# AlejandroSilvestri/os1

Measured on AMD Instinct MI355X. Metric: frames/sec extract+match, 1920x1080 @ 2000 ORB feats, higher is better.
Workload: dtype u8

## Files before the change

### os1_amd/csrc/orbfe_extractor.hip

```cpp
#include <hip/hip_runtime.h>
#include <unistd.h>
#include <sched.h>

#include <algorithm>
#include <cctype>
#include <chrono>
#include <cmath>
#include <cstdarg>
#include <cstdio>
#include <cstdlib>
#include <cstring>
#include <memory>
#include <mutex>
#include <string>
#include <thread>
#include <vector>

#include "../../include/orbfe.h"
#include "glibc_sincosf.h"
#include "host_pool.h"
#include "orbfe_internal.h"
#include "quadtree.h"

namespace orbfe {
int launch_pyramid(const PyramidParams& P, int nframes, hipStream_t st, const ConeParams* cone);
void launch_ingest(const uint8_t* src, long long sstride, uint8_t* dst, long long dpitch, int rowBytes, int rows, hipStream_t st);
void launch_to_gray(const uint8_t* const* raw, long long rawStride, const uint8_t* const* gray, long long grayPitch, int rows,
                    int cols, int channels, const int coef[3], int shift, bool aligned, int nframes, hipStream_t st);
void launch_fast(const PyramidParams& P, int nframes, hipStream_t st);
uint32_t fast_cell_geo(int wCell, int hCell);
void launch_compact(const PyramidParams& P, int nframes, hipStream_t st);
void launch_compact_local(const PyramidParams& P, int nframes, hipStream_t st, int level0, int level1);
void launch_describe(const PyramidParams& P, const SelKp* sel, int nsel, float* angle, uint8_t* desc,
                     hipStream_t st);
void launch_sincos(const float* deg, int n, float* c, float* s, hipStream_t st);
void launch_spin(unsigned long long ticks, hipStream_t st);
void launch_describe_slots(const PyramidParams& P, const SelKp* sel, int nslots, float* angle, uint8_t* desc,
                           const uint32_t* selCount, int selPerFrame, const int* selOff, hipStream_t st, bool fourWaves, float* angle2 = nullptr,
                           uint8_t* desc2 = nullptr);
int launch_quadtree(const QtParams& Q, int nframes, hipStream_t st, int ldsBudget);
int bow_launch_descend(orbfe_vocabulary* v, const uint8_t* d_desc, int n, int levelsup, uint2* d_out, hipStream_t st);
int bow_assemble(orbfe_vocabulary* v, const uint2* ln, int n, uint32_t* bow_ids, double* bow_values, int* n_words,
                 uint32_t* fv_nodes, uint32_t* fv_offsets, uint32_t* fv_features, int* n_fv_nodes,
                 uint32_t* word_of_feature, uint32_t* node_of_feature);
int bow_device(const orbfe_vocabulary* v);
void launch_sfi(const SfiParams& S, int nframes, hipStream_t st);
void launch_sfi_carry(const SfiParams& S, int lastFrame, SelKp* cSel, float* cAngle, uint8_t* cDesc, uint32_t* cCount,
                      hipStream_t st);

thread_local std::string g_err;
void set_err(const char* fmt, ...) {
  char buf[512];
  va_list ap;
  va_start(ap, fmt);
  vsnprintf(buf, sizeof buf, fmt, ap);
  va_end(ap);
  g_err = buf;
}
}

using namespace orbfe;

#define HIP_TRY(expr)                                                                        \
  do {                                                                                       \
    hipError_t e_ = (expr);                                                                  \
    if (e_ != hipSuccess) {                                                                  \
      set_err("%s failed: %s (%s:%d)", #expr, hipGetErrorString(e_), __FILE__, __LINE__);    \
      return ORBFE_ERR_HIP;                                                                  \
    }                                                                                        \
  } while (0)

namespace {
inline int cv_round_f(float v) { return (int)lrintf(v); }
inline int cv_floor_f(float v) { int i = (int)v; return i - (i > v); }
inline short sat_short(int v) { return (short)(v < -32768 ? -32768 : v > 32767 ? 32767 : v); }
inline long long align_up(long long v, long long a) { return (v + a - 1) / a * a; }
double now_ms() {
  return std::chrono::duration<double, std::milli>(std::chrono::steady_clock::now().time_since_epoch()).count();
}

template <class T>
struct DevBuf {
  T* p = nullptr;
  size_t n = 0;
  int ensure(size_t count) {
    if (count <= n) return ORBFE_OK;
    if (p) (void)hipFree(p);
    p = nullptr;
    n = 0;
    HIP_TRY(hipMalloc((void**)&p, count * sizeof(T)));
    n = count;
    return ORBFE_OK;
  }
  void release() { if (p) (void)hipFree(p); p = nullptr; n = 0; }
};
template <class T>
struct PinBuf {
  T* p = nullptr;
  size_t n = 0;
  int ensure(size_t count) {
    if (count <= n) return ORBFE_OK;
    if (p) (void)hipHostFree(p);
    p = nullptr;
    n = 0;
    HIP_TRY(hipHostMalloc((void**)&p, count * sizeof(T), hipHostMallocDefault));
    n = count;
    return ORBFE_OK;
  }
  void release() { if (p) (void)hipHostFree(p); p = nullptr; n = 0; }
};
}

struct orbfe_sfi_chain {
  int device = 0, n0cap = 0;
  DevBuf<SelKp> sel[2];
  DevBuf<float> angle[2];
  DevBuf<uint8_t> desc[2];
  DevBuf<uint32_t> count;
  hipEvent_t ready[2] = {};
  long long seq = 0;
  bool isolated = false;
  bool restart = false;
  orbfe_matcher* hostMatcher = nullptr;
  std::vector<OrbfeKeyPoint> hostPrevKps;
  std::vector<uint8_t> hostPrevDesc;
  bool hostPrevValid = false;
  ~orbfe_sfi_chain() {
    (void)hipSetDevice(device);
    if (hostMatcher) orbfe_matcher_destroy(hostMatcher);
    for (int i = 0; i < 2; i++) { sel[i].release(); angle[i].release(); desc[i].release(); if (ready[i]) (void)hipEventDestroy(ready[i]); }
    count.release();
  }
};

struct UploadLane {
  std::mutex mu;
  hipStream_t stream = nullptr;
};
static UploadLane* upload_lane(int device) {
  static std::mutex mu;
  static UploadLane* lanes[64] = {};
  if (device < 0 || device >= 64) return nullptr;
  std::lock_guard<std::mutex> lk(mu);
  if (!lanes[device]) {
    UploadLane* l = new UploadLane;
    if (hipStreamCreateWithFlags(&l->stream, hipStreamNonBlocking) != hipSuccess) { delete l; return nullptr; }
    lanes[device] = l;
  }
  return lanes[device];
}

struct orbfe_extractor {
  int nfeatures, nlevels, iniTh, minTh, device;
  double scaleFactor;
  std::vector<float> sf, isf, sigma2, isigma2;
  std::vector<int> nfeat;
  static constexpr int kMaxSub = 4;
  hipStream_t stream = nullptr;
  hipStream_t streams[kMaxSub] = {};
  static constexpr int subBatches = 4;
  hipEvent_t evUpload = nullptr;
  bool lastLocalCand = false, submitLocalCand = false;
  bool localLists = true;
  hipEvent_t evFrame0 = nullptr, evS1[kMaxSub] = {};
  int subSel[kMaxSub] = {};
  size_t candHostCap = 0;
  bool gpuQuadtree = true;
  orbfe_vocabulary* voc = nullptr;
  int vocLevelsup = 4;
  bool pendingBow = false;
  DevBuf<uint2> d_bow;
  PinBuf<uint2> h_bow;
  std::vector<std::vector<uint2>> bowKp;
  int kpPerFrameCap = 0;
  bool geomGpuQtOk = true;
  QtParams QP{};
  int selOff[kMaxLevels + 1] = {};
  int selPerFrame = 0;
  DevBuf<uint16_t> d_own;
  hipEvent_t evQt[2] = {};
  std::vector<int> frameKpBase, frameKpCount;

  int rows = 0, cols = 0, batchCap = 0;
  PyramidParams P{};
  DevBuf<uint8_t> d_tables, d_slab, d_in;
  DevBuf<ConeRange> d_coneTab, d_coneTailTab;
  ConeParams coneTail{};
  bool tailOk = false;
  int tailBase = 0, tailTile = 48;
  ConeParams cone{};
  bool coneOk = false;
  bool qtJump = true;
  int qtLdsBudget = 120 * 1024;
  int pollWaitUs = 0;
  bool zeroCopyOut = true;
  bool zeroCopyBatches = false;
  bool ingestKernel = true;
  int coneTile = 0;
  int coneMaxFrames = 2;
  DevBuf<FastCell> d_cells;
  DevBuf<uint8_t> d_zeros;
  DevBuf<uint32_t> d_cellCount, d_slots, d_cand;
  DevBuf<const uint8_t*> d_frame0;
  template <class T> struct View { T* p = nullptr; };
  DevBuf<uint8_t> d_outArena;
  PinBuf<uint8_t> h_outArena;
  size_t outArenaBytes = 0;
  View<uint32_t> d_levelStart, d_selCount, h_levelStart, h_selCount;
  View<SelKp> d_sel, h_sel;
  View<float> d_angle, h_angle;
  View<uint8_t> d_desc, h_desc;
  View<int32_t> d_m12, h_m12, d_nm, h_nm;
  DevBuf<uint16_t> d_sfiOrder;
  DevBuf<int> d_sfiOrderCount;
  DevBuf<uint32_t> d_sfiPool, d_sfiPcount;
  bool pendingMatched = false;
  DevBuf<float> d_f32tmp;
  bool profileKernels = false;
  PinBuf<const uint8_t*> h_frame0;
  PinBuf<uint32_t> h_cand;
  long long inPitch = 0;
  int inFormat = ORBFE_INPUT_GRAY8, grayVariant = ORBFE_GRAY_Q15;
  int gaussVariant = ORBFE_GAUSS_ED;
  long long grayPitch = 0;
  DevBuf<uint8_t> d_gray;
  bool inLinear = false;
  int lastFrames = 0;
  int deferredFrames = 0, deferredCap = 0;
  bool deferredMatched = false;
  std::vector<OrbfeKeyPoint> defKps;
  std::vector<uint8_t> defDesc;
  std::vector<int> defN, defNm;
  std::vector<int32_t> defM12;
  bool lastGpuQt = false, lastZeroCopy = false, submitZeroCopy = false;
  bool describe4 = true;
  float stageMs[5] = {0, 0, 0, 0, 0};
  hipEvent_t ev[kMaxSub][6] = {};
  double kernMs[5] = {0, 0, 0, 0, 0};
  long long kernBatches = 0, kernFrames = 0;

  struct Meta { int16_t x, y; uint8_t score, level; };
  struct Worker {
    QuadTree qt;
    std::vector<int16_t> qx, qy;
    std::vector<uint8_t> qs;
    std::vector<int> qsel;
  };
  std::unique_ptr<HostPool> pool;
  int hostThreads = 1;
  std::vector<Worker> workers;
  std::vector<std::vector<Meta>> taskOut;
  std::vector<Meta> meta;

  ~orbfe_extractor() {
    (void)hipSetDevice(device);
    for (auto& st : streams) if (st) (void)hipStreamSynchronize(st);
    d_bow.release(); h_bow.release();
    d_tables.release(); d_coneTab.release(); d_coneTailTab.release(); d_slab.release(); d_in.release(); d_cellCount.release();
    d_sfiOrder.release(); d_sfiOrderCount.release(); d_sfiPool.release(); d_sfiPcount.release();
    d_cells.release(); d_zeros.release(); d_slots.release(); d_cand.release(); d_frame0.release(); d_gray.release(); d_outArena.release(); h_outArena.release();
    d_f32tmp.release();
    h_frame0.release(); h_cand.release();
    for (auto& es : ev) for (auto& e : es) if (e) (void)hipEventDestroy(e);
    for (auto& e : evS1) if (e) (void)hipEventDestroy(e);
    for (auto& e : evQt) if (e) (void)hipEventDestroy(e);
    d_own.release();
    if (evFrame0) (void)hipEventDestroy(evFrame0);
    if (evUpload) (void)hipEventDestroy(evUpload);

    for (auto& st : streams) if (st) (void)hipStreamDestroy(st);
  }

  int setGeometry(int r, int c) {
    if (r == rows && c == cols) return ORBFE_OK;
    if (c > 4095 || r > 4095) {
      set_err("image %dx%d exceeds the 4095-pixel coordinate packing limit", c, r);
      return ORBFE_ERR_INVALID;
    }
    bool qtOk = true;
    int kpSum = 8;
    PyramidParams Q{};
    Q.nlevels = nlevels;
    Q.iniTh = iniTh;
// ... 306 lines not shown
      int g = f + 1;
      while (g < f0 + nf && gray[g] == gray[g - 1] + frameBytes) g++;
      HIP_TRY(hipMemcpyAsync(d_in.p + frameBytes * f, gray[f], frameBytes * (size_t)(g - f - 1) + lastBytes, hipMemcpyHostToDevice, st));
      for (int k = f; k < g; k++) devAt[k] = d_in.p + frameBytes * k;
      f = g;
    }
    return ORBFE_OK;
  }

  int uploadSlots(int f0, int nf, const uint8_t* const* gray, size_t stride, int r, int c, hipStream_t st) {
    for (int f = f0; f < f0 + nf; f++) {
      if (inLinear)
        HIP_TRY(hipMemcpyAsync(d_in.p + (size_t)inPitch * rows * f, gray[f], stride * (size_t)(r - 1) + c, hipMemcpyHostToDevice, st));
      else
        HIP_TRY(hipMemcpy2DAsync(d_in.p + (size_t)inPitch * rows * f, inPitch, gray[f], stride, c, r, hipMemcpyHostToDevice, st));
    }
    return ORBFE_OK;
  }

  int runGpuQt(int nframes, const uint8_t* const* gray, bool onDevice, int r, int c, size_t stride, OrbfeKeyPoint* kps,
               uint8_t* desc, int cap, int* n_out) {
    int rc = submitGpuQt(nframes, gray, onDevice, r, c, stride);
    if (rc) return rc;
    return waitGpuQt(kps, desc, cap, n_out);
  }

  bool submitProfiled = false, fastTimed = false;
  std::vector<const uint8_t*> devAt;
  int pendingFrames = 0;
  double tSubmit0 = 0, tSubmit1 = 0;

  struct MatchSpec { orbfe_sfi_chain* chain; float bounds[4]; int window; float nnratio; int checkOri; };

  int submitGpuQt(int nframes, const uint8_t* const* gray, bool onDevice, int r, int c, size_t stride,
                  const MatchSpec* ms = nullptr) {
    if (pendingFrames) { set_err("a submitted batch has not been collected yet"); return ORBFE_ERR_INVALID; }
    HIP_TRY(hipSetDevice(device));
    int rc;
    if ((rc = setGeometry(r, c))) return rc;
    if (!geomGpuQtOk) {
      set_err("image %dx%d: a pyramid level has more than 4 (or no) quadtree root nodes; only the blocking "
              "orbfe_extract / orbfe_extract_batch calls (host quadtree path) handle such aspect ratios", c, r);
      return ORBFE_ERR_INVALID;
    }
    if ((rc = setBatch(nframes, !onDevice, stride))) return rc;
    const double t0 = now_ms();
    hipStream_t st = streams[0];
    const int ch = inChannels();
    const int rowBytes = c * ch;
    for (int f = 0; f < nframes; f++)
      if (!gray[f]) { set_err("frame %d is NULL", f); return ORBFE_ERR_INVALID; }
    devAt.resize(nframes);
    bool pinned = !onDevice;
    std::vector<const uint8_t*>& mappedAt = devAt;
    if (!onDevice) {
      const size_t extent = stride * (size_t)(r - 1) + (size_t)rowBytes;
      const int ncheck = nframes <= coneMaxFrames ? nframes : 1;
      for (int f = 0; f < ncheck && pinned; f++) {
        void* dp = nullptr;
        void* dpEnd = nullptr;
        const bool ok = hipHostGetDevicePointer(&dp, const_cast<uint8_t*>(gray[f]), 0) == hipSuccess && dp &&
                        hipHostGetDevicePointer(&dpEnd, const_cast<uint8_t*>(gray[f]) + extent - 1, 0) == hipSuccess &&
                        (const uint8_t*)dpEnd - (const uint8_t*)dp == (ptrdiff_t)(extent - 1);
        if (!ok) { (void)hipGetLastError(); pinned = false; break; }
        mappedAt[f] = static_cast<const uint8_t*>(dp);
      }
    }
    if (!onDevice && !pinned) {
      if ((rc = uploadFrames(0, nframes, gray, stride, r, rowBytes, st, devAt.data()))) return rc;
    } else if (!onDevice && ingestKernel && nframes <= coneMaxFrames &&
               ((((uintptr_t)gray[0] | (uintptr_t)gray[nframes - 1] | (uintptr_t)stride | (uintptr_t)rowBytes) & 3) == 0)) {
      for (int f = 0; f < nframes; f++) {
        uint8_t* d = d_in.p + (size_t)inPitch * rows * f;
        launch_ingest(mappedAt[f], (long long)stride, d, inPitch, rowBytes, r, st);
        devAt[f] = d;
      }
      HIP_TRY(hipGetLastError());
    } else if (!onDevice) {
      UploadLane* lane = upload_lane(device);
      if (!lane) { set_err("cannot create the upload stream"); return ORBFE_ERR_HIP; }
      std::lock_guard<std::mutex> lk(lane->mu);
      if ((rc = uploadFrames(0, nframes, gray, stride, r, rowBytes, lane->stream, devAt.data()))) return rc;
      HIP_TRY(hipEventRecord(evUpload, lane->stream));
      HIP_TRY(hipStreamWaitEvent(st, evUpload, 0));
    }
    bool rawAligned = ((onDevice ? (long long)stride : inPitch) & 3) == 0;
    for (int f = 0; f < nframes; f++) {
      const uint8_t* raw = onDevice ? gray[f] : devAt[f];
      rawAligned = rawAligned && ((uintptr_t)raw & (ch == 4 ? 15 : 3)) == 0;
      h_frame0.p[f] = ch == 1 ? raw : d_gray.p + (size_t)grayPitch * rows * f;
      h_frame0.p[nframes + f] = raw;
    }
    const long long rawStride = onDevice ? (long long)stride : inPitch;
    P.stride0 = ch == 1 ? rawStride : grayPitch;
    P.frameBase = 0;
    P.gaussVariant = gaussVariant;
    if (ch == 1 && nframes <= 2) {
      P.frame0 = nullptr;
      P.frameInline[0] = h_frame0.p[0];
      P.frameInline[1] = h_frame0.p[nframes - 1];
    } else {
      P.frame0 = d_frame0.p;
      HIP_TRY(hipMemcpyAsync(d_frame0.p, h_frame0.p, sizeof(void*) * nframes * (ch == 1 ? 1 : 2), hipMemcpyHostToDevice, st));
    }
    if (ch > 1) {
      const bool q15 = grayVariant == ORBFE_GRAY_Q15;
      const int cr = q15 ? 9798 : 4899, cg = q15 ? 19235 : 9617, cb = q15 ? 3735 : 1868;
      const bool rgb = inFormat == ORBFE_INPUT_RGB8 || inFormat == ORBFE_INPUT_RGBA8;
      const int coef[3] = {rgb ? cr : cb, cg, rgb ? cb : cr};
      launch_to_gray(d_frame0.p + nframes, rawStride, d_frame0.p, grayPitch, r, c, ch, coef, q15 ? 15 : 14, rawAligned, nframes, st);
    }
    const bool prof = profileKernels;
    QP.cand = d_cand.p; QP.levelStart = d_levelStart.p; QP.candCap = P.candCap; QP.nlevels = nlevels; QP.frameBase = 0;
    QP.own = d_own.p;
    QP.sel = d_sel.p; QP.selCount = d_selCount.p; QP.selPerFrame = selPerFrame;
    const bool small = nframes <= coneMaxFrames;
    const bool zeroCopy = zeroCopyOut && small && !voc && !(ms && ms->chain);
    submitZeroCopy = zeroCopy;
    QP.jump = qtJump ? 1 : 0;
    const bool kernelOut = zeroCopyBatches && !small;
    QP.selHost = (zeroCopy || kernelOut) ? h_sel.p : nullptr;
    QP.selCountHost = (zeroCopy || kernelOut) ? h_selCount.p : nullptr;
    for (int l = 0; l < nlevels; l++) {
      QP.levW[l] = P.lv[l].w; QP.levH[l] = P.lv[l].h; QP.nfeat[l] = nfeat[l]; QP.selOff[l] = selOff[l];
      QP.candBase[l] = P.lv[l].slotBase;
    }
    float* angOut = zeroCopy ? h_angle.p : d_angle.p;
    uint8_t* descOut = zeroCopy ? h_desc.p : d_desc.p;
    const int qtLds = small ? qtLdsBudget : 0;
    const bool four = describe4 && small;
    const bool localCand = small && localLists;
    submitLocalCand = localCand;
    QP.levelLocal = localCand ? 1 : 0;
    {
      if (prof) HIP_TRY(hipEventRecord(ev[0][0], st));
      if (launch_pyramid(P, nframes, st, coneOk && small ? &cone : (tailOk && !small ? &coneTail : nullptr))) { set_err("cannot configure the pyramid kernel"); return ORBFE_ERR_HIP; }
      const bool timeFast = prof || !small;
      fastTimed = timeFast;
      if (timeFast) HIP_TRY(hipEventRecord(ev[0][1], st));
      launch_fast(P, nframes, st);
      if (timeFast) HIP_TRY(hipEventRecord(ev[0][2], st));
      if (localCand) launch_compact_local(P, nframes, st, 0, nlevels);
      else launch_compact(P, nframes, st);
      if (prof) HIP_TRY(hipEventRecord(ev[0][3], st));
      if (prof) HIP_TRY(hipEventRecord(evQt[0], st));
      if (launch_quadtree(QP, nframes, st, qtLds)) { set_err("cannot configure the quadtree kernel"); return ORBFE_ERR_HIP; }
      if (prof) HIP_TRY(hipEventRecord(evQt[1], st));
      if (prof) HIP_TRY(hipEventRecord(ev[0][4], st));
      launch_describe_slots(P, d_sel.p, nframes * selPerFrame, angOut, descOut, d_selCount.p, selPerFrame, selOff, st, four,
                            kernelOut ? h_angle.p : nullptr, kernelOut ? h_desc.p : nullptr);
      if (prof) HIP_TRY(hipEventRecord(ev[0][5], st));
      HIP_TRY(hipGetLastError());
    }
    const int nslots = nframes * selPerFrame;
    pendingBow = false;
    if (voc) {
      if ((rc = d_bow.ensure(nslots)) || (rc = h_bow.ensure(nslots))) return rc;
      if ((rc = bow_launch_descend(voc, d_desc.p, nslots, vocLevelsup, d_bow.p, st))) return rc;
      HIP_TRY(hipMemcpyAsync(h_bow.p, d_bow.p, sizeof(uint2) * nslots, hipMemcpyDeviceToHost, st));
      pendingBow = true;
    }
    pendingMatched = false;
    if (ms && ms->chain) {
      orbfe_sfi_chain& ch = *ms->chain;
      const int n0cap = selOff[1] - selOff[0];
      if (ch.n0cap != n0cap || ch.device != device) { set_err("match chain belongs to a different extractor configuration"); return ORBFE_ERR_INVALID; }
      if ((rc = d_sfiOrder.ensure((size_t)batchCap * n0cap))) return rc;
      if ((rc = d_sfiOrderCount.ensure(batchCap))) return rc;
      if ((rc = d_sfiPool.ensure((size_t)batchCap * n0cap * n0cap))) return rc;
      if ((rc = d_sfiPcount.ensure((size_t)batchCap * n0cap))) return rc;
      SfiParams SP{};
      SP.sel = d_sel.p; SP.angle = d_angle.p; SP.desc = d_desc.p; SP.selCount = d_selCount.p;
      SP.selPerFrame = selPerFrame; SP.n0cap = n0cap; SP.frameBase = 0;
      const int prev = (int)((ch.seq + 1) & 1), cur = (int)(ch.seq & 1);
      SP.carrySel = ch.sel[prev].p; SP.carryAngle = ch.angle[prev].p; SP.carryDesc = ch.desc[prev].p;
      const bool iso = ch.isolated;
      SP.carryCount = ch.count.p + ((ch.seq == 0 || iso || ch.restart) ? 2 : prev);
      ch.restart = false;
      SP.minX = ms->bounds[0]; SP.minY = ms->bounds[2];
      SP.invW = static_cast<float>(64) / static_cast<float>(ms->bounds[1] - ms->bounds[0]);
      SP.invH = static_cast<float>(48) / static_cast<float>(ms->bounds[3] - ms->bounds[2]);
      SP.window = (float)ms->window; SP.nnratio = ms->nnratio; SP.checkOri = ms->checkOri;
      SP.order = d_sfiOrder.p; SP.orderCount = d_sfiOrderCount.p; SP.pool = d_sfiPool.p; SP.pcount = d_sfiPcount.p;
      SP.matches12 = kernelOut ? h_m12.p : d_m12.p; SP.nmatches = kernelOut ? h_nm.p : d_nm.p;
      if (ch.seq > 0 && !iso) HIP_TRY(hipStreamWaitEvent(st, ch.ready[prev], 0));
      launch_sfi(SP, nframes, st);
      HIP_TRY(hipGetLastError());
      if (!iso) {
        launch_sfi_carry(SP, nframes - 1, ch.sel[cur].p, ch.angle[cur].p, ch.desc[cur].p, ch.count.p + cur, st);
        HIP_TRY(hipGetLastError());
        HIP_TRY(hipEventRecord(ch.ready[cur], st));
      }
      ch.seq++;
      pendingMatched = true;
    }
    if (!zeroCopy && !kernelOut) HIP_TRY(hipMemcpyAsync(h_outArena.p, d_outArena.p, outArenaBytes, hipMemcpyDeviceToHost, st));
    submitProfiled = prof;
    tSubmit0 = t0;
    tSubmit1 = now_ms();
    pendingFrames = nframes;
    return ORBFE_OK;
  }

  int waitOnly() {
    if (!pendingFrames) return ORBFE_OK;
    HIP_TRY(hipSetDevice(device));
    hipStream_t st = streams[0];
    if (pollWaitUs > 0) {
      hipError_t q;
      while ((q = hipStreamQuery(st)) == hipErrorNotReady) usleep((useconds_t)pollWaitUs);
      if (q != hipSuccess) HIP_TRY(q);
    }
    HIP_TRY(hipStreamSynchronize(st));
    return ORBFE_OK;
  }

  int waitGpuQt(OrbfeKeyPoint* kps, uint8_t* desc, int cap, int* n_out, int32_t* matches12 = nullptr,
                int* nmatches = nullptr) {
    if (!pendingFrames) { set_err("no submitted batch to collect"); return ORBFE_ERR_INVALID; }
    HIP_TRY(hipSetDevice(device));
    const int nframes = pendingFrames;
    pendingFrames = 0;
    hipStream_t st = streams[0];
    const double t0 = tSubmit0, t1 = tSubmit1;
    const double t1b = now_ms();
    if (pollWaitUs > 0) {
      hipError_t q;
      while ((q = hipStreamQuery(st)) == hipErrorNotReady) usleep((useconds_t)pollWaitUs);
      if (q != hipSuccess) HIP_TRY(q);
    }
    HIP_TRY(hipStreamSynchronize(st));
    const double t2 = now_ms();
    {
      float ms = 0;
      if (fastTimed && hipEventElapsedTime(&ms, ev[0][1], ev[0][2]) == hipSuccess) kernMs[1] += ms;
      if (submitProfiled) {
        if (hipEventElapsedTime(&ms, ev[0][0], ev[0][1]) == hipSuccess) kernMs[0] += ms;
        if (hipEventElapsedTime(&ms, ev[0][2], ev[0][3]) == hipSuccess) kernMs[2] += ms;
        if (hipEventElapsedTime(&ms, ev[0][4], ev[0][5]) == hipSuccess) kernMs[3] += ms;
        if (hipEventElapsedTime(&ms, evQt[0], evQt[1]) == hipSuccess) kernMs[4] += ms;
      }
      if (fastTimed) {
        kernBatches++;
        kernFrames += nframes;
      }
    }
    int status = ORBFE_OK;
    if (pendingBow) bowKp.resize(nframes);
    else bowKp.clear();
    for (int f = 0; f < nframes; f++) {
      OrbfeKeyPoint* ko = kps + (size_t)f * cap;
      uint8_t* dout = desc + (size_t)f * cap * 32;
      if (pendingBow) bowKp[f].clear();
      int n = 0;
      for (int l = 0; l < nlevels; l++) {
        const int cnt = (int)h_selCount.p[(size_t)f * kMaxLevels + l];
        const size_t base = (size_t)f * selPerFrame + selOff[l];
        const float scale = sf[l];
        const float size = (float)(int)(31 * sf[l]);
        for (int i = 0; i < cnt; i++) {
          if (n >= cap) { n++; continue; }
          const SelKp s = h_sel.p[base + i];
          OrbfeKeyPoint kp;
          kp.x = (float)(s.xy & 0xffff);
          kp.y = (float)(s.xy >> 16);
          if (l != 0) { kp.x *= scale; kp.y *= scale; }
          kp.size = size;
          kp.angle = h_angle.p[base + i];
          kp.response = (float)(s.lf >> 24);
          kp.octave = l;
          kp.class_id = -1;
          ko[n] = kp;
          memcpy(dout + (size_t)n * 32, h_desc.p + (base + i) * 32, 32);
          if (pendingBow) bowKp[f].push_back(h_bow.p[base + i]);
          n++;
        }
      }
      n_out[f] = n;
      if (n > cap) {
        set_err("frame %d produced %d keypoints, cap is %d", f, n, cap);
        status = ORBFE_ERR_OVERFLOW;
      }
    }
    if (matches12 && nmatches) {
      const int n0cap = selOff[1] - selOff[0];
      for (int f = 0; f < nframes; f++) {
        int32_t* row = matches12 + (size_t)f * cap;
        const int m = std::min(cap, n0cap);
        if (pendingMatched) {
          memcpy(row, h_m12.p + (size_t)f * n0cap, sizeof(int32_t) * m);
          nmatches[f] = h_nm.p[f];
        } else {
          nmatches[f] = 0;
        }
        for (int i = pendingMatched ? m : 0; i < cap; i++) row[i] = -1;
      }
    }
    const double t3 = now_ms();
    stageMs[0] = (float)(t1 - t0);
    stageMs[1] = (float)(t2 - t1b);
    stageMs[2] = 0;
    stageMs[3] = (float)(t3 - t2);
    stageMs[4] = (float)(t3 - t0);
    lastFrames = nframes;
    lastGpuQt = true;
    lastZeroCopy = submitZeroCopy;
    lastLocalCand = submitLocalCand;
    return status;
  }

  int run(int nframes, const uint8_t* const* gray, bool onDevice, int r, int c, size_t stride, OrbfeKeyPoint* kps,
          uint8_t* desc, int cap, int* n_out) {
    if (pendingFrames) { set_err("a submitted batch has not been collected yet"); return ORBFE_ERR_INVALID; }
    HIP_TRY(hipSetDevice(device));
    int rc;
    if ((rc = setGeometry(r, c))) return rc;
    if ((rc = setBatch(nframes, !onDevice, stride))) return rc;
    const double t0 = now_ms();
    if (!pool) {
      pool.reset(new HostPool(hostThreads));
      workers.resize(hostThreads);
    }
    if (inChannels() != 1) { set_err("colour input needs the GPU quadtree path (unset ORBFE_HOST_QUADTREE)"); return ORBFE_ERR_INVALID; }
    const int nsub = std::min(nframes, std::min(kMaxSub, std::max(1, subBatches)));
    const int maxKp = kpPerFrameCap;
    if ((rc = ensureSubStreams(nsub))) return rc;
    int subF0[kMaxSub + 1];
    for (int s = 0; s <= nsub; s++) subF0[s] = (int)((long long)nframes * s / nsub);

    devAt.resize(nframes);
    for (int f = 0; f < nframes; f++) {
      if (!gray[f]) { set_err("frame %d is NULL", f); return ORBFE_ERR_INVALID; }
      h_frame0.p[f] = onDevice ? gray[f] : d_in.p + (size_t)inPitch * rows * f;
    }
    P.stride0 = onDevice ? (long long)stride : inPitch;
    P.gaussVariant = gaussVariant;
    P.frame0 = d_frame0.p;
    HIP_TRY(hipMemcpyAsync(d_frame0.p, h_frame0.p, sizeof(void*) * nframes, hipMemcpyHostToDevice, streams[0]));
    HIP_TRY(hipEventRecord(evFrame0, streams[0]));
    for (int s = 0; s < nsub; s++) {
      hipStream_t st = streams[s];
      const int f0 = subF0[s], nf = subF0[s + 1] - f0;
      if (s) HIP_TRY(hipStreamWaitEvent(st, evFrame0, 0));
      if (!onDevice && (rc = uploadSlots(f0, nf, gray, stride, r, c, st))) return rc;
      PyramidParams Q = P;
// ... 516 lines not shown
  if (v && !h->gpuQuadtree) { set_err("the fused bag-of-words path needs the GPU quadtree path"); return ORBFE_ERR_INVALID; }
  h->voc = v;
  h->vocLevelsup = levelsup;
  return ORBFE_OK;
}

int orbfe_extract_bow(orbfe_extractor* h, int frame, uint32_t* bow_ids, double* bow_values, int* n_words, uint32_t* fv_nodes,
                      uint32_t* fv_offsets, uint32_t* fv_features, int* n_fv_nodes, uint32_t* word_of_feature,
                      uint32_t* node_of_feature) {
  if (!h || !bow_ids || !bow_values || !n_words || !fv_nodes || !fv_offsets || !fv_features || !n_fv_nodes) {
    set_err("bad argument");
    return ORBFE_ERR_INVALID;
  }
  if (!h->voc || frame < 0 || frame >= (int)h->bowKp.size()) {
    set_err("no bag-of-words result for frame %d (set a vocabulary before extracting)", frame);
    return ORBFE_ERR_INVALID;
  }
  const std::vector<uint2>& ln = h->bowKp[frame];
  return bow_assemble(h->voc, ln.data(), (int)ln.size(), bow_ids, bow_values, n_words, fv_nodes, fv_offsets, fv_features,
                      n_fv_nodes, word_of_feature, node_of_feature);
}

int orbfe_extract_bow_raw(orbfe_extractor* h, int frame, uint32_t* leaf_node, uint32_t* level_node, int cap, int* n_out) {
  if (!h || !leaf_node || !level_node || !n_out || cap < 0) { set_err("bad argument"); return ORBFE_ERR_INVALID; }
  if (!h->voc || frame < 0 || frame >= (int)h->bowKp.size()) {
    set_err("no bag-of-words result for frame %d (set a vocabulary before extracting)", frame);
    return ORBFE_ERR_INVALID;
  }
  const std::vector<uint2>& ln = h->bowKp[frame];
  *n_out = (int)ln.size();
  const int m = std::min(cap, (int)ln.size());
  for (int i = 0; i < m; i++) { leaf_node[i] = ln[i].x; level_node[i] = ln[i].y; }
  return ORBFE_OK;
}

int orbfe_extractor_max_keypoints_for_size(const orbfe_extractor* h, int rows, int cols) {
  if (!h || rows <= 0 || cols <= 0) return 0;
  int n = 0;
  for (int l = 0; l < h->nlevels; l++) {
    const int w = cv_round_f((float)cols * h->isf[l]), hh = cv_round_f((float)rows * h->isf[l]);
    int roots = hh > 2 * kBorder ? (int)roundf(static_cast<float>(w - 2 * kBorder) / (hh - 2 * kBorder)) : 0;
    if (roots < 0) roots = 0;
    n += std::max(h->nfeat[l] + 2, 4 * roots);
  }
  return n;
}

int orbfe_extract_batch(orbfe_extractor* h, int nframes, const uint8_t* const* gray, int in_device_memory, int rows,
                        int cols, size_t stride_bytes, OrbfeKeyPoint* kps, uint8_t* desc, int cap, int* n_out) {
  if (!h || !n_out) { set_err("NULL argument"); return ORBFE_ERR_INVALID; }
  if (nframes <= 0) return ORBFE_OK;
  for (int f = 0; f < nframes; f++) n_out[f] = 0;
  if (rows == 0 || cols == 0 || !gray) return ORBFE_OK;
  if (rows < 0 || cols < 0 || stride_bytes < (size_t)cols * h->inChannels() || !kps || !desc || cap <= 0) {
    set_err("invalid image / output arguments");
    return ORBFE_ERR_INVALID;
  }
  if (h->pendingFrames) { set_err("a submitted batch has not been collected yet"); return ORBFE_ERR_INVALID; }
  {
    HIP_TRY(hipSetDevice(h->device));
    const int rc = h->setGeometry(rows, cols);
    if (rc) return rc;
  }
  if (h->gpuQuadtree && h->geomGpuQtOk)
    return h->runGpuQt(nframes, gray, in_device_memory != 0, rows, cols, stride_bytes, kps, desc, cap, n_out);
  return h->run(nframes, gray, in_device_memory != 0, rows, cols, stride_bytes, kps, desc, cap, n_out);
}

static bool gpu_route_ok(orbfe_extractor* h, int rows, int cols, int* rc) {
  *rc = ORBFE_OK;
  if (!h->gpuQuadtree) return false;
  if (hipSetDevice(h->device) != hipSuccess) { set_err("hipSetDevice failed"); *rc = ORBFE_ERR_HIP; return false; }
  if (h->pendingFrames || h->deferredFrames) return true;
  *rc = h->setGeometry(rows, cols);
  return *rc == ORBFE_OK && h->geomGpuQtOk;
}

static int deferred_extract(orbfe_extractor* h, int nframes, const uint8_t* const* gray, int in_device_memory, int rows, int cols,
                            size_t stride_bytes) {
  if (h->pendingFrames || h->deferredFrames) { set_err("a submitted batch has not been collected yet"); return ORBFE_ERR_INVALID; }
  const int cap = orbfe_extractor_max_keypoints_for_size(h, rows, cols);
  h->deferredCap = cap;
  h->defKps.resize((size_t)nframes * cap);
  h->defDesc.resize((size_t)nframes * cap * 32);
  h->defN.assign(nframes, 0);
  const int rc = orbfe_extract_batch(h, nframes, gray, in_device_memory, rows, cols, stride_bytes, h->defKps.data(), h->defDesc.data(),
                                     cap, h->defN.data());
  if (rc) return rc;
  h->deferredFrames = nframes;
  h->deferredMatched = false;
  return ORBFE_OK;
}

static int deferred_collect(orbfe_extractor* h, OrbfeKeyPoint* kps, uint8_t* desc, int cap, int* n_out, int32_t* matches12,
                            int* nmatches) {
  const int nframes = h->deferredFrames, dcap = h->deferredCap;
  h->deferredFrames = 0;
  int status = ORBFE_OK;
  for (int f = 0; f < nframes; f++) {
    const int n = h->defN[f];
    n_out[f] = n;
    if (n > cap) { set_err("frame %d produced %d keypoints, cap is %d", f, n, cap); status = ORBFE_ERR_OVERFLOW; }
    const int m = std::min(n, cap);
    memcpy(kps + (size_t)f * cap, h->defKps.data() + (size_t)f * dcap, sizeof(OrbfeKeyPoint) * (size_t)m);
    memcpy(desc + (size_t)f * cap * 32, h->defDesc.data() + (size_t)f * dcap * 32, 32 * (size_t)m);
    if (matches12 && nmatches) {
      int32_t* row = matches12 + (size_t)f * cap;
      for (int i = 0; i < cap; i++) row[i] = -1;
      nmatches[f] = 0;
      if (h->deferredMatched) {
        memcpy(row, h->defM12.data() + (size_t)f * dcap, sizeof(int32_t) * (size_t)std::min(cap, dcap));
        nmatches[f] = h->defNm[f];
      }
    }
  }
  return status;
}

int orbfe_extract_batch_submit(orbfe_extractor* h, int nframes, const uint8_t* const* gray, int in_device_memory,
                               int rows, int cols, size_t stride_bytes) {
  if (!h || !gray || nframes <= 0 || rows <= 0 || cols <= 0 || stride_bytes < (size_t)cols * h->inChannels()) {
    set_err("invalid arguments");
    return ORBFE_ERR_INVALID;
  }
  int rc;
  if (!gpu_route_ok(h, rows, cols, &rc)) {
    if (rc) return rc;
    return deferred_extract(h, nframes, gray, in_device_memory, rows, cols, stride_bytes);
  }
  if (h->deferredFrames) { set_err("a submitted batch has not been collected yet"); return ORBFE_ERR_INVALID; }
  return h->submitGpuQt(nframes, gray, in_device_memory != 0, rows, cols, stride_bytes);
}

int orbfe_extract_batch_wait(orbfe_extractor* h) {
  if (!h) { set_err("invalid arguments"); return ORBFE_ERR_INVALID; }
  if (h->deferredFrames) return ORBFE_OK;
  return h->waitOnly();
}

int orbfe_extract_batch_collect(orbfe_extractor* h, OrbfeKeyPoint* kps, uint8_t* desc, int cap, int* n_out) {
  if (!h || !kps || !desc || !n_out || cap <= 0) { set_err("invalid arguments"); return ORBFE_ERR_INVALID; }
  if (h->deferredFrames) return deferred_collect(h, kps, desc, cap, n_out, nullptr, nullptr);
  return h->waitGpuQt(kps, desc, cap, n_out);
}

int orbfe_sfi_chain_create(const orbfe_extractor* h, orbfe_sfi_chain** out) {
  if (!h || !out) { set_err("NULL argument"); return ORBFE_ERR_INVALID; }
  *out = nullptr;
  HIP_TRY(hipSetDevice(h->device));
  orbfe_sfi_chain* c = new orbfe_sfi_chain();
  c->device = h->device;
  c->n0cap = h->selOff[1] - h->selOff[0];
  int rc = ORBFE_OK;
  for (int i = 0; i < 2 && rc == ORBFE_OK; i++) {
    if ((rc = c->sel[i].ensure(c->n0cap))) break;
    if ((rc = c->angle[i].ensure(c->n0cap))) break;
    if ((rc = c->desc[i].ensure((size_t)c->n0cap * 32))) break;
    if (hipEventCreateWithFlags(&c->ready[i], hipEventDisableTiming) != hipSuccess) { set_err("hipEventCreate failed"); rc = ORBFE_ERR_HIP; }
  }
  if (rc == ORBFE_OK) rc = c->count.ensure(4);
  if (rc == ORBFE_OK) {
    const uint32_t init[4] = {0xffffffffu, 0xffffffffu, 0xffffffffu, 0xffffffffu};
    if (hipMemcpy(c->count.p, init, sizeof init, hipMemcpyHostToDevice) != hipSuccess) { set_err("hipMemcpy failed"); rc = ORBFE_ERR_HIP; }
  }
  if (rc != ORBFE_OK) { delete c; return rc; }
  *out = c;
  return ORBFE_OK;
}

void orbfe_sfi_chain_destroy(orbfe_sfi_chain* c) { delete c; }

int orbfe_sfi_chain_set_isolated(orbfe_sfi_chain* c, int isolated) {
  if (!c) { set_err("chain is NULL"); return ORBFE_ERR_INVALID; }
  if (c->isolated != (isolated != 0)) {
    c->seq = 0;
    c->hostPrevValid = false;
  }
  c->isolated = isolated != 0;
  return ORBFE_OK;
}

int orbfe_sfi_chain_restart(orbfe_sfi_chain* c) {
  if (!c) { set_err("chain is NULL"); return ORBFE_ERR_INVALID; }
  c->restart = true;
  return ORBFE_OK;
}

int orbfe_extract_batch_submit_matched(orbfe_extractor* h, orbfe_sfi_chain* chain, int nframes, const uint8_t* const* gray,
                                       int in_device_memory, int rows, int cols, size_t stride_bytes, const float bounds[4],
                                       int window_size, float nnratio, int check_orientation) {
  if (!h || !chain || !gray || !bounds || nframes <= 0 || rows <= 0 || cols <= 0 || stride_bytes < (size_t)cols * h->inChannels() || window_size <= 0) {
    set_err("invalid arguments");
    return ORBFE_ERR_INVALID;
  }
  int rc;
  if (!gpu_route_ok(h, rows, cols, &rc)) {
    if (rc) return rc;
    if ((rc = deferred_extract(h, nframes, gray, in_device_memory, rows, cols, stride_bytes))) return rc;
    if (!chain->hostMatcher && (rc = orbfe_matcher_create(h->device, &chain->hostMatcher))) { h->deferredFrames = 0; return rc; }
    const int cap = h->deferredCap;
    h->defM12.assign((size_t)nframes * cap, -1);
    h->defNm.assign(nframes, 0);
    std::vector<const OrbfeKeyPoint*> k1, k2;
    std::vector<const uint8_t*> d1, d2;
    std::vector<int> n1, n2, frameOf, nm;
    std::vector<std::vector<float>> pxy;
    std::vector<float*> prev;
    std::vector<int32_t*> m12;
    for (int f = 0; f < nframes; f++) {
      const OrbfeKeyPoint* pk;
      const uint8_t* pd;
      int pn;
      if (f == 0) {
        if (!chain->hostPrevValid || chain->isolated || chain->restart) continue;
        pk = chain->hostPrevKps.data(); pd = chain->hostPrevDesc.data(); pn = (int)chain->hostPrevKps.size();
      } else {
        pk = h->defKps.data() + (size_t)(f - 1) * cap; pd = h->defDesc.data() + (size_t)(f - 1) * cap * 32; pn = h->defN[f - 1];
      }
      pxy.emplace_back((size_t)std::max(pn, 1) * 2);
      for (int j = 0; j < pn; j++) { pxy.back()[2 * j] = pk[j].x; pxy.back()[2 * j + 1] = pk[j].y; }
      k1.push_back(pk); d1.push_back(pd); n1.push_back(pn);
      k2.push_back(h->defKps.data() + (size_t)f * cap); d2.push_back(h->defDesc.data() + (size_t)f * cap * 32); n2.push_back(h->defN[f]);
      m12.push_back(h->defM12.data() + (size_t)f * cap);
      frameOf.push_back(f);
    }
    for (auto& v : pxy) prev.push_back(v.data());
    nm.assign(k1.size(), 0);
    if (!k1.empty()) {
      rc = orbfe_search_for_initialization_batch(chain->hostMatcher, (int)k1.size(), k1.data(), d1.data(), n1.data(), k2.data(), d2.data(),
                                                 n2.data(), bounds, prev.data(), m12.data(), window_size, nnratio, check_orientation,
                                                 nm.data());
      if (rc) { h->deferredFrames = 0; return rc; }
      for (size_t p = 0; p < frameOf.size(); p++) h->defNm[frameOf[p]] = nm[p];
    }
    const int last = nframes - 1, ln = h->defN[last];
    chain->hostPrevKps.assign(h->defKps.begin() + (size_t)last * cap, h->defKps.begin() + (size_t)last * cap + ln);
    chain->hostPrevDesc.assign(h->defDesc.begin() + (size_t)last * cap * 32, h->defDesc.begin() + ((size_t)last * cap + ln) * 32);
    chain->hostPrevValid = !chain->isolated;
    chain->restart = false;
    h->deferredMatched = true;
    return ORBFE_OK;
  }
  if (h->deferredFrames) { set_err("a submitted batch has not been collected yet"); return ORBFE_ERR_INVALID; }
  orbfe_extractor::MatchSpec ms;
  ms.chain = chain;
  memcpy(ms.bounds, bounds, sizeof ms.bounds);
  ms.window = window_size;
  ms.nnratio = nnratio;
  ms.checkOri = check_orientation;
  return h->submitGpuQt(nframes, gray, in_device_memory != 0, rows, cols, stride_bytes, &ms);
}

int orbfe_extract_batch_collect_matched(orbfe_extractor* h, OrbfeKeyPoint* kps, uint8_t* desc, int cap, int* n_out,
                                        int32_t* matches12, int* nmatches) {
  if (!h || !kps || !desc || !n_out || !matches12 || !nmatches || cap <= 0) { set_err("invalid arguments"); return ORBFE_ERR_INVALID; }
  if (h->deferredFrames) return deferred_collect(h, kps, desc, cap, n_out, matches12, nmatches);
  return h->waitGpuQt(kps, desc, cap, n_out, matches12, nmatches);
}

int orbfe_extract(orbfe_extractor* h, const uint8_t* gray, int rows, int cols, size_t stride_bytes, OrbfeKeyPoint* kps,
                  uint8_t* desc, int cap, int* n_out) {
  if (!n_out) { set_err("n_out is NULL"); return ORBFE_ERR_INVALID; }
  *n_out = 0;
  if (!gray || rows == 0 || cols == 0) return ORBFE_OK;
  const uint8_t* frames[1] = {gray};
  return orbfe_extract_batch(h, 1, frames, 0, rows, cols, stride_bytes, kps, desc, cap, n_out);
}

int orbfe_debug_level_size(const orbfe_extractor* h, int level, int* w, int* hgt) {
  if (!h || level < 0 || level >= h->nlevels || h->rows == 0) { set_err("bad level / no frame yet"); return ORBFE_ERR_INVALID; }
  *w = h->P.lv[level].w;
  *hgt = h->P.lv[level].h;
  return ORBFE_OK;
}

int orbfe_debug_level_copy(orbfe_extractor* h, int frame, int level, uint8_t* out) {
  if (!h || level < 0 || level >= h->nlevels || frame < 0 || frame >= h->lastFrames) {
    set_err("bad frame/level");
    return ORBFE_ERR_INVALID;
  }
  HIP_TRY(hipSetDevice(h->device));
  const LevelGeom& L = h->P.lv[level];
  const uint8_t* src;
  size_t pitch;
  if (level == 0) {
    src = h->h_frame0.p[frame];
    pitch = (size_t)h->P.stride0;
  } else {
    src = h->d_slab.p + (size_t)h->P.slabBytes * frame + L.off;
    pitch = L.pitch;
  }
  HIP_TRY(hipMemcpy2D(out, L.w, src, pitch, L.w, L.h, hipMemcpyDeviceToHost));
  return ORBFE_OK;
}

int orbfe_debug_candidates(orbfe_extractor* h, int frame, int level, int32_t* xys, int cap, int* n_out) {
  if (!h || !n_out || level < 0 || level >= h->nlevels || frame < 0 || frame >= h->lastFrames) {
    set_err("bad frame/level");
    return ORBFE_ERR_INVALID;
  }
  HIP_TRY(hipSetDevice(h->device));
  uint32_t ls[kMaxLevels + 1];
  HIP_TRY(hipMemcpy(ls, h->d_levelStart.p + (size_t)frame * (kMaxLevels + 1), sizeof(ls), hipMemcpyDeviceToHost));
  const size_t start = h->lastLocalCand ? (size_t)h->P.lv[level].slotBase : (size_t)ls[level];
  const int n = h->lastLocalCand ? (int)ls[level] : (int)(ls[level + 1] - ls[level]);
  *n_out = n;
  if (n <= 0 || !xys) return ORBFE_OK;
  std::vector<uint32_t> tmp(n);
  HIP_TRY(hipMemcpy(tmp.data(), h->d_cand.p + (size_t)h->P.candCap * frame + start, sizeof(uint32_t) * n,
                    hipMemcpyDeviceToHost));
  for (int i = 0; i < n && i < cap; i++) {
    xys[3 * i] = (int)(tmp[i] & 0xfff) - kBorder;
    xys[3 * i + 1] = (int)((tmp[i] >> 12) & 0xfff) - kBorder;
    xys[3 * i + 2] = (int)(tmp[i] >> 24);
  }
// ... 73 lines not shown
```

### os1_amd/csrc/orbfe_sfi.hip

```cpp
#include <hip/hip_runtime.h>

#include <cstdlib>

#include "orbfe_internal.h"

namespace orbfe {

constexpr int kSfiGridCols = 64, kSfiGridRows = 48;
constexpr int kSfiThLow = 50, kSfiHisto = 30;

struct SfiFrame {
  const SelKp* sel;
  const float* angle;
  const uint8_t* desc;
  int n;
};

__device__ __forceinline__ SfiFrame sfi_frame(const SfiParams& S, int f) {
  SfiFrame F;
  if (f < 0) {
    F.sel = S.carrySel; F.angle = S.carryAngle; F.desc = S.carryDesc;
    F.n = S.carryCount ? (int)*S.carryCount : -1;
    if (F.n > S.n0cap) F.n = -1;
  } else {
// ... 224 lines not shown
  }
  __syncthreads();
  int cur = 0, rounds = 0;
  for (;;) {
    const int* M = Mbuf[cur];
    int* Mn = Mbuf[cur ^ 1];
    for (int i = tid; i < n2; i += kSfiThreads) head[i] = -1;
    __syncthreads();
    for (int j = tid; j < n1; j += kSfiThreads) {
      const int m = M[j];
      if (m >= 0) next[j] = atomicExch(&head[m & 0xffff], j);
    }
    __syncthreads();
    int changed = 0;
    for (int i1 = tid; i1 < n1; i1 += kSfiThreads) {
      const int cnt = pcnt[i1];
      int bestDist = 0x7fffffff, bestDist2 = 0x7fffffff, bestIdx2 = -1;
      for (int c = 0; c < cnt; c++) {
        const uint32_t entry = inLds ? lpool[off[i1] + c] : gpool[(long long)i1 * cap + c];
        const int i2 = (int)(entry & 0xffff), dist = (int)(entry >> 16);
        int vmd = 0x7fffffff;
        for (int j = head[i2]; j >= 0; j = next[j])
          if (j < i1) vmd = min(vmd, M[j] >> 16);
        if (vmd <= dist) continue;
        if (dist < bestDist) { bestDist2 = bestDist; bestDist = dist; bestIdx2 = i2; }
        else if (dist < bestDist2) bestDist2 = dist;
      }
      int m = -1;
      if (bestDist <= kSfiThLow && (float)bestDist < (float)bestDist2 * S.nnratio) m = bestIdx2 | (bestDist << 16);
      Mn[i1] = m;
      changed |= m != M[i1];
    }
    const int any = __syncthreads_or(changed);
    cur ^= 1;
    if (!any) break;
    if (++rounds >= maxRounds) {
      dbgSerial = 1;
      int* M2 = Mbuf[cur];
      int* vmd = head;
      for (int i = tid; i < n2; i += kSfiThreads) vmd[i] = 0x7fffffff;
      __syncthreads();
      if (tid < 64) {
        if (inLds) sfi_serial_outcomes(tid, n1, pcnt, [&](int q, int c) { return lpool[off[q] + c]; }, S.nnratio, vmd, M2);
        else sfi_serial_outcomes(tid, n1, pcnt, [&](int q, int c) { return gpool[(long long)q * cap + c]; }, S.nnratio, vmd, M2);
      }
      __syncthreads();
      for (int i = tid; i < n2; i += kSfiThreads) head[i] = -1;
      __syncthreads();
      for (int j = tid; j < n1; j += kSfiThreads) {
        const int m = M2[j];
        if (m >= 0) next[j] = atomicExch(&head[m & 0xffff], j);
      }
      __syncthreads();
      break;
    }
  }
  const int* M = Mbuf[cur];
  int* vn12 = Mbuf[cur ^ 1];
  int* binOf = off;
  __syncthreads();
  for (int j = tid; j < n1; j += kSfiThreads) {
    const int m = M[j];
    int v = -1, bin = -1;
    if (m >= 0) {
      const int i2 = m & 0xffff;
      bool last = true;
      for (int k = head[i2]; k >= 0; k = next[k]) last = last && k <= j;
      if (last) v = i2;
      if (S.checkOri) {
        bin = sfi_rot_bin(F1.angle[j], F2.angle[i2]);
        atomicAdd(&hist[bin], 1);
      }
    }
    vn12[j] = v;
    binOf[j] = bin;
  }
  __syncthreads();
  int ind1 = -1, ind2 = -1, ind3 = -1;
  if (S.checkOri) {
    int max1 = 0, max2 = 0, max3 = 0;
    for (int i = 0; i < kSfiHisto; i++) {
      const int s = hist[i];
      if (s > max1) { max3 = max2; max2 = max1; max1 = s; ind3 = ind2; ind2 = ind1; ind1 = i; }
      else if (s > max2) { max3 = max2; max2 = s; ind3 = ind2; ind2 = i; }
      else if (s > max3) { max3 = s; ind3 = i; }
    }
    if (max2 < 0.1f * (float)max1) { ind2 = -1; ind3 = -1; }
    else if (max3 < 0.1f * (float)max1) { ind3 = -1; }
  }
  int nm = 0;
  for (int i = tid; i < cap; i += kSfiThreads) {
    int v = -1;
    if (i < n1) {
      v = vn12[i];
      const int b = binOf[i];
      if (S.checkOri && b >= 0 && b != ind1 && b != ind2 && b != ind3) v = -1;
    }
    out[i] = v;
    nm += v >= 0;
  }
#pragma unroll
  for (int o = 32; o > 0; o >>= 1) nm += __shfl_xor(nm, o, 64);
  if ((tid & 63) == 0 && nm) atomicAdd(&misc[0], nm);
  __syncthreads();
  if (tid == 0) S.nmatches[f] = misc[0];
  if (g_sfiDbg && tid == 0) {
    const int r = atomicAdd(&g_sfiDbg[0], 1);
    if (r < kSfiDbgRecords) {
      int* rec = g_sfiDbg + 8 + 8 * r;
      rec[0] = f; rec[1] = rounds; rec[2] = total; rec[3] = dbgSerial;
      rec[4] = (int)(__builtin_amdgcn_s_memtime() - tStart); rec[5] = n1; rec[6] = n2; rec[7] = inLds;
    }
  }
}

static int* s_sfiDbg = nullptr;
static void sfi_debug_setup() {
  static bool done = false;
  if (done) return;
  done = true;
  if (!ORBFE_EXP_ENV("ORBFE_SFI_DEBUG")) return;
  if (hipMalloc((void**)&s_sfiDbg, sizeof(int) * (8 + 8 * kSfiDbgRecords)) != hipSuccess) { s_sfiDbg = nullptr; return; }
  (void)hipMemset(s_sfiDbg, 0, sizeof(int) * (8 + 8 * kSfiDbgRecords));
  (void)hipMemcpyToSymbol(HIP_SYMBOL(g_sfiDbg), &s_sfiDbg, sizeof s_sfiDbg);
}
int sfi_debug_read(int* out, int capRecords, int reset) {
  if (!s_sfiDbg) return 0;
  int n = 0;
  if (hipMemcpy(&n, s_sfiDbg, sizeof(int), hipMemcpyDeviceToHost) != hipSuccess) return -1;
  n = std::min(std::min(n, kSfiDbgRecords), capRecords);
  if (n > 0 && hipMemcpy(out, s_sfiDbg + 8, sizeof(int) * 8 * (size_t)n, hipMemcpyDeviceToHost) != hipSuccess) return -1;
  if (reset) (void)hipMemset(s_sfiDbg, 0, sizeof(int));
  return n;
}

__global__ __launch_bounds__(256) void k_sfi_carry(SfiParams S, int lastFrame, SelKp* cSel, float* cAngle, uint8_t* cDesc,
                                                   uint32_t* cCount) {
  const long long base = (long long)lastFrame * S.selPerFrame;
  const int i = blockIdx.x * 256 + threadIdx.x;
  if (i < S.n0cap) {
    cSel[i] = S.sel[base + i];
    cAngle[i] = S.angle[base + i];
  }
  if (i < S.n0cap * 8)
    reinterpret_cast<uint32_t*>(cDesc)[i] = reinterpret_cast<const uint32_t*>(S.desc + base * 32)[i];
  if (i == 0) *cCount = S.selCount[(long long)lastFrame * kMaxLevels];
}

void launch_sfi_carry(const SfiParams& S, int lastFrame, SelKp* cSel, float* cAngle, uint8_t* cDesc, uint32_t* cCount,
                      hipStream_t st) {
  hipLaunchKernelGGL(k_sfi_carry, dim3((S.n0cap * 8 + 255) / 256), dim3(256), 0, st, S, lastFrame, cSel, cAngle, cDesc, cCount);
}

void launch_sfi(const SfiParams& S, int nframes, hipStream_t st) {
  sfi_debug_setup();
  hipLaunchKernelGGL(k_sfi_sort, dim3(nframes), dim3(256), sizeof(int) * 3 * S.n0cap, st, S);
  hipLaunchKernelGGL(k_sfi_candidates, dim3(S.n0cap, nframes), dim3(64), 0, st, S);
  const int fixedWords = 6 * S.n0cap + 1 + 32 + 2;
  int ldsPool = (60 * 1024 / 4) - fixedWords;
  if (ldsPool > 8192) ldsPool = 8192;
  if (const char* e = ORBFE_EXP_ENV("ORBFE_SFI_LDS_POOL")) ldsPool = std::min(ldsPool, std::max(0, atoi(e)));
  if (ldsPool < 0) ldsPool = 0;
  int maxRounds = 32;
  if (const char* e = getenv("ORBFE_SFI_MAX_ROUNDS")) maxRounds = atoi(e) < 1 ? 1 : atoi(e);
  static const int threads = [] { const char* e = ORBFE_EXP_ENV("ORBFE_SFI_THREADS"); return e ? atoi(e) : 512; }();
  if (threads == 256)
    hipLaunchKernelGGL(k_sfi_resolve<256>, dim3(nframes), dim3(256), sizeof(int) * (fixedWords + ldsPool), st, S, ldsPool, maxRounds);
  else
    hipLaunchKernelGGL(k_sfi_resolve<512>, dim3(nframes), dim3(512), sizeof(int) * (fixedWords + ldsPool), st, S, ldsPool, maxRounds);
}

}
```

Baseline: 89530.

## Use a ring of carry slots so batches chain without serializing on matching

Replaces the double-buffered inter-batch carry with a 12-slot ring. The carry of the last frame is now written right after description, and each slot has a readersDone event. The SFI launch is split into sort and match so that only the match stage waits on the previous batch's carry-ready event. This lets concurrent batches on different streams overlap more of their sort and match work, at the cost of more device buffers and events.

```diff
diff --git a/os1_amd/csrc/orbfe_extractor.hip b/os1_amd/csrc/orbfe_extractor.hip
--- a/os1_amd/csrc/orbfe_extractor.hip
+++ b/os1_amd/csrc/orbfe_extractor.hip
@@ -44,7 +44,8 @@
                  uint32_t* fv_nodes, uint32_t* fv_offsets, uint32_t* fv_features, int* n_fv_nodes,
                  uint32_t* word_of_feature, uint32_t* node_of_feature);
 int bow_device(const orbfe_vocabulary* v);
-void launch_sfi(const SfiParams& S, int nframes, hipStream_t st);
+void launch_sfi_sort(const SfiParams& S, int nframes, hipStream_t st);
+void launch_sfi_match(const SfiParams& S, int nframes, hipStream_t st);
 void launch_sfi_carry(const SfiParams& S, int lastFrame, SelKp* cSel, float* cAngle, uint8_t* cDesc, uint32_t* cCount,
                       hipStream_t st);
 
@@ -111,14 +112,17 @@
 };
 }
 
+constexpr int kSfiCarrySlots = 12;
 struct orbfe_sfi_chain {
   int device = 0, n0cap = 0;
-  DevBuf<SelKp> sel[2];
-  DevBuf<float> angle[2];
-  DevBuf<uint8_t> desc[2];
+  DevBuf<SelKp> sel[kSfiCarrySlots];
+  DevBuf<float> angle[kSfiCarrySlots];
+  DevBuf<uint8_t> desc[kSfiCarrySlots];
   DevBuf<uint32_t> count;
-  hipEvent_t ready[2] = {};
+  hipEvent_t ready[kSfiCarrySlots] = {};
+  hipEvent_t readersDone[kSfiCarrySlots] = {};
   long long seq = 0;
+  long long head = 0;
   bool isolated = false;
   bool restart = false;
   orbfe_matcher* hostMatcher = nullptr;
@@ -128,7 +132,11 @@
   ~orbfe_sfi_chain() {
     (void)hipSetDevice(device);
     if (hostMatcher) orbfe_matcher_destroy(hostMatcher);
-    for (int i = 0; i < 2; i++) { sel[i].release(); angle[i].release(); desc[i].release(); if (ready[i]) (void)hipEventDestroy(ready[i]); }
+    for (int i = 0; i < kSfiCarrySlots; i++) {
+      sel[i].release(); angle[i].release(); desc[i].release();
+      if (ready[i]) (void)hipEventDestroy(ready[i]);
+      if (readersDone[i]) (void)hipEventDestroy(readersDone[i]);
+    }
     count.release();
   }
 };
@@ -741,6 +749,29 @@
       if (prof) HIP_TRY(hipEventRecord(ev[0][5], st));
       HIP_TRY(hipGetLastError());
     }
+    const bool chained = ms && ms->chain;
+    SfiParams SP{};
+    int carryPrev = -1;
+    if (chained) {
+      orbfe_sfi_chain& ch = *ms->chain;
+      const int n0cap = selOff[1] - selOff[0];
+      if (ch.n0cap != n0cap || ch.device != device) { set_err("match chain belongs to a different extractor configuration"); return ORBFE_ERR_INVALID; }
+      if ((rc = d_sfiOrder.ensure((size_t)batchCap * n0cap))) return rc;
+      if ((rc = d_sfiOrderCount.ensure(batchCap))) return rc;
+      if ((rc = d_sfiPool.ensure((size_t)batchCap * n0cap * n0cap))) return rc;
+      if ((rc = d_sfiPcount.ensure((size_t)batchCap * n0cap))) return rc;
+      SP.sel = d_sel.p; SP.angle = d_angle.p; SP.desc = d_desc.p; SP.selCount = d_selCount.p;
+      SP.selPerFrame = selPerFrame; SP.n0cap = n0cap; SP.frameBase = 0;
+      if (!ch.isolated) {
+        const int cur = (int)(ch.head % kSfiCarrySlots);
+        if (ch.head > 0) carryPrev = (int)((ch.head - 1) % kSfiCarrySlots);
+        HIP_TRY(hipStreamWaitEvent(st, ch.readersDone[cur], 0));
+        launch_sfi_carry(SP, nframes - 1, ch.sel[cur].p, ch.angle[cur].p, ch.desc[cur].p, ch.count.p + cur, st);
+        HIP_TRY(hipGetLastError());
+        HIP_TRY(hipEventRecord(ch.ready[cur], st));
+        ch.head++;
+      }
+    }
     const int nslots = nframes * selPerFrame;
     pendingBow = false;
     if (voc) {
@@ -750,21 +781,11 @@
       pendingBow = true;
     }
     pendingMatched = false;
-    if (ms && ms->chain) {
+    if (chained) {
       orbfe_sfi_chain& ch = *ms->chain;
-      const int n0cap = selOff[1] - selOff[0];
-      if (ch.n0cap != n0cap || ch.device != device) { set_err("match chain belongs to a different extractor configuration"); return ORBFE_ERR_INVALID; }
-      if ((rc = d_sfiOrder.ensure((size_t)batchCap * n0cap))) return rc;
-      if ((rc = d_sfiOrderCount.ensure(batchCap))) return rc;
-      if ((rc = d_sfiPool.ensure((size_t)batchCap * n0cap * n0cap))) return rc;
-      if ((rc = d_sfiPcount.ensure((size_t)batchCap * n0cap))) return rc;
-      SfiParams SP{};
-      SP.sel = d_sel.p; SP.angle = d_angle.p; SP.desc = d_desc.p; SP.selCount = d_selCount.p;
-      SP.selPerFrame = selPerFrame; SP.n0cap = n0cap; SP.frameBase = 0;
-      const int prev = (int)((ch.seq + 1) & 1), cur = (int)(ch.seq & 1);
-      SP.carrySel = ch.sel[prev].p; SP.carryAngle = ch.angle[prev].p; SP.carryDesc = ch.desc[prev].p;
-      const bool iso = ch.isolated;
-      SP.carryCount = ch.count.p + ((ch.seq == 0 || iso || ch.restart) ? 2 : prev);
+      const bool reads = carryPrev >= 0 && ch.seq > 0 && !ch.restart;
+      if (carryPrev >= 0) { SP.carrySel = ch.sel[carryPrev].p; SP.carryAngle = ch.angle[carryPrev].p; SP.carryDesc = ch.desc[carryPrev].p; }
+      SP.carryCount = ch.count.p + (reads ? carryPrev : kSfiCarrySlots);
       ch.restart = false;
       SP.minX = ms->bounds[0]; SP.minY = ms->bounds[2];
       SP.invW = static_cast<float>(64) / static_cast<float>(ms->bounds[1] - ms->bounds[0]);
@@ -772,14 +793,11 @@
       SP.window = (float)ms->window; SP.nnratio = ms->nnratio; SP.checkOri = ms->checkOri;
       SP.order = d_sfiOrder.p; SP.orderCount = d_sfiOrderCount.p; SP.pool = d_sfiPool.p; SP.pcount = d_sfiPcount.p;
       SP.matches12 = kernelOut ? h_m12.p : d_m12.p; SP.nmatches = kernelOut ? h_nm.p : d_nm.p;
-      if (ch.seq > 0 && !iso) HIP_TRY(hipStreamWaitEvent(st, ch.ready[prev], 0));
-      launch_sfi(SP, nframes, st);
+      launch_sfi_sort(SP, nframes, st);
+      if (carryPrev >= 0) HIP_TRY(hipStreamWaitEvent(st, ch.ready[carryPrev], 0));
+      launch_sfi_match(SP, nframes, st);
       HIP_TRY(hipGetLastError());
-      if (!iso) {
-        launch_sfi_carry(SP, nframes - 1, ch.sel[cur].p, ch.angle[cur].p, ch.desc[cur].p, ch.count.p + cur, st);
-        HIP_TRY(hipGetLastError());
-        HIP_TRY(hipEventRecord(ch.ready[cur], st));
-      }
+      if (carryPrev >= 0) HIP_TRY(hipEventRecord(ch.readersDone[carryPrev], st));
       ch.seq++;
       pendingMatched = true;
     }
@@ -1602,15 +1620,17 @@
   c->device = h->device;
   c->n0cap = h->selOff[1] - h->selOff[0];
   int rc = ORBFE_OK;
-  for (int i = 0; i < 2 && rc == ORBFE_OK; i++) {
+  for (int i = 0; i < kSfiCarrySlots && rc == ORBFE_OK; i++) {
     if ((rc = c->sel[i].ensure(c->n0cap))) break;
     if ((rc = c->angle[i].ensure(c->n0cap))) break;
     if ((rc = c->desc[i].ensure((size_t)c->n0cap * 32))) break;
-    if (hipEventCreateWithFlags(&c->ready[i], hipEventDisableTiming) != hipSuccess) { set_err("hipEventCreate failed"); rc = ORBFE_ERR_HIP; }
-  }
-  if (rc == ORBFE_OK) rc = c->count.ensure(4);
+    if (hipEventCreateWithFlags(&c->ready[i], hipEventDisableTiming) != hipSuccess ||
+        hipEventCreateWithFlags(&c->readersDone[i], hipEventDisableTiming) != hipSuccess) { set_err("hipEventCreate failed"); rc = ORBFE_ERR_HIP; }
+  }
+  if (rc == ORBFE_OK) rc = c->count.ensure(kSfiCarrySlots + 1);
   if (rc == ORBFE_OK) {
-    const uint32_t init[4] = {0xffffffffu, 0xffffffffu, 0xffffffffu, 0xffffffffu};
+    uint32_t init[kSfiCarrySlots + 1];
+    for (uint32_t& v : init) v = 0xffffffffu;
     if (hipMemcpy(c->count.p, init, sizeof init, hipMemcpyHostToDevice) != hipSuccess) { set_err("hipMemcpy failed"); rc = ORBFE_ERR_HIP; }
   }
   if (rc != ORBFE_OK) { delete c; return rc; }
diff --git a/os1_amd/csrc/orbfe_sfi.hip b/os1_amd/csrc/orbfe_sfi.hip
--- a/os1_amd/csrc/orbfe_sfi.hip
+++ b/os1_amd/csrc/orbfe_sfi.hip
@@ -400,9 +400,12 @@
   hipLaunchKernelGGL(k_sfi_carry, dim3((S.n0cap * 8 + 255) / 256), dim3(256), 0, st, S, lastFrame, cSel, cAngle, cDesc, cCount);
 }
 
-void launch_sfi(const SfiParams& S, int nframes, hipStream_t st) {
+void launch_sfi_sort(const SfiParams& S, int nframes, hipStream_t st) {
+  hipLaunchKernelGGL(k_sfi_sort, dim3(nframes), dim3(256), sizeof(int) * 3 * S.n0cap, st, S);
+}
+
+void launch_sfi_match(const SfiParams& S, int nframes, hipStream_t st) {
   sfi_debug_setup();
-  hipLaunchKernelGGL(k_sfi_sort, dim3(nframes), dim3(256), sizeof(int) * 3 * S.n0cap, st, S);
   hipLaunchKernelGGL(k_sfi_candidates, dim3(S.n0cap, nframes), dim3(64), 0, st, S);
   const int fixedWords = 6 * S.n0cap + 1 + 32 + 2;
   int ldsPool = (60 * 1024 / 4) - fixedWords;
```

New measurement: 89350. About the same (-0.2%).
